# unibas-gravis/icp-proposal

Measured on AMD Instinct MI355X. Metric: ICP-proposal MH iterations/sec (femur GPMM r=50, ~50k-vtx target), higher is better.
Workload: dtype f64

## Files before the change

### icp-proposal_amd/csrc/icp_dense.hpp

```cpp
#pragma once
#include "icp_kernels.hpp"

namespace icp {

constexpr int kLdsDoubles = 18432;


__device__ __forceinline__ void write_corr(const CorrBuffers& cb, int k, int id, int aux, d3 pt, bool keep, d3 n,
                                           const Pose& pose, const double* __restrict__ ref, const double* __restrict__ mean) {
  double v0 = (pt.x - pose.t[0]) - pose.ctr[0], v1 = (pt.y - pose.t[1]) - pose.ctr[1], v2 = (pt.z - pose.t[2]) - pose.ctr[2];
  double b0 = ((pose.R[0] * v0 + pose.R[3] * v1) + pose.R[6] * v2) + pose.ctr[0];
  double b1 = ((pose.R[1] * v0 + pose.R[4] * v1) + pose.R[7] * v2) + pose.ctr[1];
  double b2 = ((pose.R[2] * v0 + pose.R[5] * v1) + pose.R[8] * v2) + pose.ctr[2];
  cb.id[k] = id;
  cb.aux[k] = aux;
  cb.pt[3 * k] = pt.x; cb.pt[3 * k + 1] = pt.y; cb.pt[3 * k + 2] = pt.z;
  cb.keep[k] = keep ? 1 : 0;
  cb.nhat[3 * k] = n.x; cb.nhat[3 * k + 1] = n.y; cb.nhat[3 * k + 2] = n.z;
  cb.e[3 * k] = (b0 - ref[3 * id]) - mean[3 * id];
  cb.e[3 * k + 1] = (b1 - ref[3 * id + 1]) - mean[3 * id + 1];
  cb.e[3 * k + 2] = (b2 - ref[3 * id + 2]) - mean[3 * id + 2];
}


__device__ __forceinline__ void correspond_model_one(const CorrTask& c, int k, d3 cp) {
  int aux = c.nnv ? c.nnv[k] : -1;
  bool on_boundary = (c.nnv && aux >= 0) ? c.boundary[aux] != 0 : false;
  d3 n = vertex_normal(c.x, c.tris, c.adj_off, c.adj, k);
  write_corr(c.cb, k, k, aux, cp, c.boundary_aware ? !on_boundary : true, n, c.pose, c.ref, c.mean);
}

__device__ __forceinline__ void correspond_target_one(const CorrTask& c, int k, int id) {
  bool on_boundary = c.boundary[id] != 0;
// ... 489 lines not shown
  const int tid = threadIdx.x, tw = 1 << tw_log2, ty = tid >> tw_log2, tx = tid & (tw - 1);
  const int rows = n + extra;
  for (int j = 0; j < n; ++j) {
    const double ajj = W[(size_t)j * ld + j];
    if (!(ajj > 0.0)) return false;
    const double inv = fast_rcp(ajj);
    for (int i = j + 1 + ty; i < rows; i += tw) {
      const double uij = W[(size_t)i * ld + j] * inv;
      const int kmax = i < n ? i : n - 1;
      for (int k = j + 1 + tx; k <= kmax; k += tw) W[(size_t)i * ld + k] = fma(-uij, W[(size_t)k * ld + j], W[(size_t)i * ld + k]);
    }
    __syncthreads();
  }
  return true;
}


#ifdef ICP_EIGEN_TIMING
extern __device__ long long g_eigen_stamps[64];
#define FAC_STAMP(i) do { if (threadIdx.x == 0 && blockIdx.x == 0) g_eigen_stamps[i] = __builtin_amdgcn_s_memrealtime(); } while (0)
#else
#define FAC_STAMP(i)
#endif

typedef double dense2 __attribute__((ext_vector_type(2)));

static __host__ __device__ inline int factor_tile_count(int r) {
  const int tr = (r + 2) >> 1;
  int c = 0;
  for (int t = 0; t < tr; ++t) c += (t >> 1) + 1;
  return c;
}

template <int TPT, int NT>
__device__ __forceinline__ bool factor_reg_body(int r, const double* __restrict__ Mpart, int S, double* __restrict__ M,
                                                double* __restrict__ alpha_out, int* __restrict__ status, int tail_base = -1,
                                                const double* __restrict__ tail_Ginv = nullptr, const double* __restrict__ Mplain = nullptr,
                                                bool solve = true) {
  __shared__ __attribute__((aligned(16))) double s_col[2][520];
  __shared__ double s_dinv[512], s_v[512];
  const int tid = threadIdx.x, n = r + 1;
  const int ld = r | 1;
  double* W = s_dyn;
  FAC_STAMP(16);
  constexpr int kGinvPer = 16;
  double ginv[kGinvPer];
  if (tail_base >= 0) {
#pragma unroll
    for (int u = 0; u < kGinvPer; ++u) {
      const int e = tid + u * NT;
      ginv[u] = e < r * r ? tail_Ginv[e] : 0.0;
    }
  }
  const int n_tiles = factor_tile_count(r);
  double v[TPT][2][4];
  int R0[TPT], C0[TPT];
#pragma unroll
  for (int t = 0; t < TPT; ++t) {
    const int e = tid + NT * t;
    int ti = 0, base = 0;
    if (e < n_tiles) {
      while (base + (ti >> 1) + 1 <= e) { base += (ti >> 1) + 1; ++ti; }
    }
    R0[t] = e < n_tiles ? 2 * ti : -2;
    C0[t] = e < n_tiles ? 4 * (e - base) : 0;
    bool live[2][4];
    size_t off[2][4];
// ... 23 lines not shown
#pragma unroll
      for (int u = 0; u < 4; ++u)
#pragma unroll
        for (int a = 0; a < 2; ++a)
#pragma unroll
          for (int c = 0; c < 4; ++c) p[u][a][c] = Mpart[(size_t)(sp + u) * nn + off[a][c]];
#pragma unroll
      for (int u = 0; u < 4; ++u)
#pragma unroll
        for (int a = 0; a < 2; ++a)
#pragma unroll
          for (int c = 0; c < 4; ++c) v[t][a][c] += p[u][a][c];
    }
    for (; sp < S; ++sp) {
      const double* P = Mpart + (size_t)sp * nn;
#pragma unroll
      for (int a = 0; a < 2; ++a)
#pragma unroll
        for (int c = 0; c < 4; ++c) v[t][a][c] += P[off[a][c]];
    }
#pragma unroll
    for (int a = 0; a < 2; ++a)
#pragma unroll
      for (int c = 0; c < 4; ++c) {
        const int i = R0[t] + a, k = C0[t] + c;
        double x = live[a][c] ? v[t][a][c] : 0.0;
        if (live[a][c]) {
          if (i < r && !Mplain) {
            if (i == k) x += 1.0;
            M[(size_t)i * r + k] = x;
            M[(size_t)k * r + i] = x;
            if (tail_base >= 0) { s_dyn[tail_base + i * ld + k] = x; s_dyn[tail_base + k * ld + i] = x; }
          }
          if (k == 0) { s_col[0][i] = x; W[(size_t)i * ld] = x; }
        }
        v[t][a][c] = x;
      }
  }
  if (tail_base >= 0) {
    const int offG = tail_base + r * ld;
#pragma unroll
    for (int u = 0; u < kGinvPer; ++u) {
      const int e = tid + u * NT;
      if (e < r * r) { const int i = e / r; s_dyn[offG + i * ld + (e - i * r)] = ginv[u]; }
    }
    for (int e = tid + kGinvPer * NT; e < r * r; e += NT) { const int i = e / r; s_dyn[offG + i * ld + (e - i * r)] = tail_Ginv[e]; }
  }
  __syncthreads();
  FAC_STAMP(17);
  bool ok = true;
  for (int j4 = 0; j4 < r && ok; j4 += 4) {
#pragma unroll
    for (int cc = 0; cc < 4; ++cc) {
      const int j = j4 + cc;
      if (j >= r) break;
      const double* cur = s_col[cc & 1];
      double* nxt = s_col[(cc + 1) & 1];
      const double ajj = cur[j];
      dense2 u[TPT], k01[TPT], k23[TPT];
#pragma unroll
      for (int t = 0; t < TPT; ++t) {
        const int rr = R0[t] < 0 ? 0 : R0[t];
        u[t] = *(const dense2*)&cur[rr];
        k01[t] = *(const dense2*)&cur[C0[t]];
        k23[t] = *(const dense2*)&cur[C0[t] + 2];
      }
      if (!(ajj > 0.0)) { ok = false; break; }
      const double inv = fast_rcp(ajj);
      const int kp = j + 1;
#pragma unroll
      for (int t = 0; t < TPT; ++t) {
        const double m0 = -(u[t].x * inv), m1 = -(u[t].y * inv);
        v[t][0][0] = fma(m0, k01[t].x, v[t][0][0]); v[t][0][1] = fma(m0, k01[t].y, v[t][0][1]);
        v[t][0][2] = fma(m0, k23[t].x, v[t][0][2]); v[t][0][3] = fma(m0, k23[t].y, v[t][0][3]);
        v[t][1][0] = fma(m1, k01[t].x, v[t][1][0]); v[t][1][1] = fma(m1, k01[t].y, v[t][1][1]);
        v[t][1][2] = fma(m1, k23[t].x, v[t][1][2]); v[t][1][3] = fma(m1, k23[t].y, v[t][1][3]);
        constexpr int cp = 0;
        (void)cp;
        if (kp < r && R0[t] >= 0 && C0[t] == (kp & ~3)) {
          const double p0 = v[t][0][(cc + 1) & 3], p1 = v[t][1][(cc + 1) & 3];
          *(dense2*)&nxt[R0[t]] = dense2{p0, p1};
          if (R0[t] >= kp && R0[t] < n) W[(size_t)R0[t] * ld + kp] = p0;
          if (R0[t] + 1 >= kp && R0[t] + 1 < n) W[(size_t)(R0[t] + 1) * ld + kp] = p1;
// ... 305 lines not shown
```

### icp-proposal_amd/csrc/icp_kernels.hpp

```cpp
#pragma once
#include <hip/hip_runtime.h>
#include <stdint.h>
#include "icp_device.hpp"

#include <cstdlib>
#include <vector>

namespace icp {

inline const char* dev_env(const char* name) {
#if defined(ICP_DEV_SWITCHES) || defined(ICP_TEST_HOOKS)
  return std::getenv(name);
#else
  (void)name;
  return nullptr;
#endif
}

constexpr int kBlock = 256;
__host__ __device__ static inline int cdiv(int a, int b) { return (a + b - 1) / b; }
static inline void set_dyn_lds(const void* fn, size_t bytes) {
  if (bytes > 48 * 1024) (void)hipFuncSetAttribute(fn, hipFuncAttributeMaxDynamicSharedMemorySize, (int)bytes);
}
static inline void set_dyn_lds_once(const void* fn, size_t max_bytes, bool* done) {
// ... 141 lines not shown
  const double* tpts;
  const unsigned char* boundary;
  const int* nnv;
  int boundary_aware;
  Pose pose;
  const double* ref;
  const double* mean;
  const int* tris;
  const int* adj_off;
  const int* adj;
  const double* cp = nullptr;
};

struct EntryInit { const double* coeffs_src = nullptr; double* coeffs_dst = nullptr; int r = 0; int* status = nullptr; };
void launch_correspond_model(hipStream_t st, int K, const double* x, const double* cp, const int* nnv,
                             const unsigned char* tgt_boundary, int boundary_aware, const Pose& pose,
                             const double* ref, const double* mean, const int* tris, const int* adj_off,
                             const int* adj, const CorrBuffers& cb, const EntryInit& init = EntryInit{});
void launch_correspond_target(hipStream_t st, int K, const double* x, const double* tpts, const int* nn_id,
                              const unsigned char* model_boundary, int boundary_aware, const Pose& pose,
                              const double* ref, const double* mean, const int* tris, const int* adj_off,
                              const int* adj, const CorrBuffers& cb, const EntryInit& init = EntryInit{});

int regression_splits(int K);
int regression_fold(int K, int r, int n_posteriors_in_launch);
int regression_macro(int r, int fold);
int regression_units(int r, int leaves, int fold, int macro);
void launch_regression(hipStream_t st, int K, int r, const double* Q, const CorrBuffers& cb, double w_tangent,
                       double kappa, double* Mpart, int* splits_out);

struct PosteriorFactorIO { const double* Mpart; int splits; double* M; double* alpha; int* status; double* scratch ;
                           double* Lout = nullptr; double* Sout = nullptr;  };
void launch_posterior_factor(hipStream_t st, int r, int n_post, const PosteriorFactorIO* io);
int posterior_factor_max();
void launch_sum_partials(hipStream_t st, int r, double* Mpart, int splits);
void launch_assemble_posterior_matrix(hipStream_t st, int r, const double* Mpart_summed, double* M);

struct TransitionTailIO {
  const double* alpha; const double* M; const double* c_from; const double* c_to; double step; double* out; int* status;
  const int* relay_in = nullptr; int* relay_out = nullptr;
};
void launch_transition_tails(hipStream_t st, int r, int n, const TransitionTailIO* io, const double* Ginv, double sigma2);
void launch_transition_tail_direct(hipStream_t st, int r, const TransitionTailIO& io, const double* G, double sigma2, double* work );

size_t eigen_work_doubles(int r);
constexpr int kEigenGaveUp = 3;
struct EigenSpec { int splits; const int* cancel; int seq; const int* ready; int ready_seq;
                   long long* wait_ticks = nullptr;  };
bool eigen_speculation_supported(int r);
struct EigenRequest { const double* M; const double* Vwarm; double* V; double* Vt; double* S; double* work; int* status;
                      const EigenSpec* spec; int* host_status; int* done_word; int done_value;
                      const double* sqrt_lambda = nullptr;
                      bool root = false;  };
constexpr int kEigenPairMax = 4;
bool launch_posterior_eigen_pair(hipStream_t st, int r, const double* sqrt_lambda, int n, const EigenRequest* rq);
struct EigenProblem {
  const double* M; const double* Vwarm ; double* Vout; double* Vtout; double* Sout; int* status;
  double* rotlog; int* meta; double* vpos; EigenSpec spec; int launch_id; int* host_status; int* done_word; int done_value;
  const double* sqrt_lambda;
};
EigenProblem eigen_problem_of(int r, const EigenRequest& rq);
void launch_posterior_eigen_resident(hipStream_t st, int r, int n, const EigenProblem* records, const int* skip, int root);
size_t eigen_many_record_bytes(int n);
int launch_posterior_eigen_many(hipStream_t st, int r, int n, const EigenRequest* rq, void* pinned_records, int* arrive);
void eigen_debug_dump(const double* work, int r);
void launch_posterior_eigen(hipStream_t st, int r, const double* M, const double* sqrt_lambda, const double* Vwarm, double* V,
// ... 724 lines not shown
```

### icp-proposal_amd/csrc/kernels_eigen.hip

```cpp
#include <algorithm>
#include <atomic>
#include <cstdio>
#include <cstdlib>

#include "icp_kernels.hpp"
#include "icp_dense.hpp"

namespace icp {

#ifdef ICP_EIGEN_TIMING
__device__ long long g_eigen_stamps[64];
#define EIG_STAMP(i) do { if (threadIdx.x == 0) g_eigen_stamps[i] = __builtin_amdgcn_s_memrealtime(); } while (0)
#else
#define EIG_STAMP(i)
#endif
}
#include "icp_tridiag.hpp"
namespace icp {

namespace {

constexpr int kEigenMaxSweeps = 40;
#ifndef ICP_LOOSE_TAU
#define ICP_LOOSE_TAU 5e-7
// ... 1372 lines not shown
  const EigenSpec spec = pb.spec;
  EIG_STAMP(0);
  if (tid == 0) s_cancel = 0;
  __syncthreads();
  if (tid == NT - 1) {
    if (spec.ready) {
      const long long t0 = __builtin_amdgcn_s_memrealtime();
      for (;;) {
        if (__hip_atomic_load(spec.ready, __ATOMIC_ACQUIRE, __HIP_MEMORY_SCOPE_AGENT) - spec.ready_seq >= 0) break;
        if (spec.cancel && __hip_atomic_load(spec.cancel, __ATOMIC_RELAXED, __HIP_MEMORY_SCOPE_SYSTEM) == spec.seq) { s_cancel = 1; break; }
        if (__builtin_amdgcn_s_memrealtime() - t0 > 500000) { s_cancel = 2; break; }
        __builtin_amdgcn_s_sleep(32);
      }
      if (spec.wait_ticks) atomicAdd((unsigned long long*)spec.wait_ticks, (unsigned long long)(__builtin_amdgcn_s_memrealtime() - t0));
    } else if (spec.cancel) {
      if (__hip_atomic_load(spec.cancel, __ATOMIC_RELAXED, __HIP_MEMORY_SCOPE_SYSTEM) == spec.seq) s_cancel = 1;
    }
  }
  __syncthreads();
  __builtin_amdgcn_fence(__ATOMIC_ACQUIRE, "agent");
  if (s_cancel) {
    if (tid == 0) {
      if (s_cancel == 2) {
        if (pb.host_status) __hip_atomic_store(pb.host_status, kEigenGaveUp, __ATOMIC_RELAXED, __HIP_MEMORY_SCOPE_SYSTEM);
        pb.Vout[0] = __builtin_nan("");
      }
      __threadfence();
      if (pb.done_word) __hip_atomic_store(pb.done_word, pb.done_value, __ATOMIC_RELEASE, __HIP_MEMORY_SCOPE_AGENT);
    }
    return;
  }
  EIG_STAMP(1);
  double* scratch = pb.rotlog;
  const bool ok = factor_reg_body<1, NT>(r, pb.M, spec.splits, scratch, scratch + (size_t)r * r, (int*)(scratch + (size_t)r * r + r),
                                         -1, nullptr, spec.splits > 0 ? nullptr : pb.M, false);
  EIG_STAMP(3);
  const int ld = r | 1;
  const double* W = s_dyn;
  if (ok) {
    for (int e = tid; e < r * r; e += NT) {
      const int i = e / r, k = e - i * r;
      const double v = k <= i ? W[(size_t)i * ld + k] * fast_rsqrt(W[(size_t)k * ld + k]) : 0.0;
      pb.Vout[(size_t)i * r + k] = v;
      pb.Vtout[(size_t)k * r + i] = v;
    }
    if (tid < r) pb.Sout[tid] = fast_rsqrt(W[(size_t)tid * ld + tid]);
  }
  EIG_STAMP(4);
  if (tid == 0) {
    pb.status[0] = ok ? 0 : 2; pb.status[-1] = 0;
    if (pb.host_status) __hip_atomic_store(pb.host_status, ok ? 0 : 2, __ATOMIC_RELAXED, __HIP_MEMORY_SCOPE_SYSTEM);
  }
  __threadfence();
  __syncthreads();
  if (tid == 0 && pb.done_word) __hip_atomic_store(pb.done_word, pb.done_value, __ATOMIC_RELEASE, __HIP_MEMORY_SCOPE_AGENT);
  EIG_STAMP(5);
}

namespace {
template <class Batch>
void launch_root_batch(hipStream_t st, int r, int n, const Batch& batch) {
  ProfScope _ps(st, KID_EIGEN);
  const size_t shmem = sizeof(double) * (size_t)(r + 1) * (r | 1);
  if (factor_tile_count(r) <= 256) {
    set_dyn_lds((const void*)k_posterior_root<Batch, 256>, shmem);
    hipLaunchKernelGGL((k_posterior_root<Batch, 256>), dim3(n), dim3(256), shmem, st, r, batch);
  } else {
// ... 94 lines not shown
```

### icp-proposal_amd/csrc/kernels_factor.hip

```cpp
#include <algorithm>

#include "icp_kernels.hpp"
#include "icp_dense.hpp"

namespace icp {

namespace {

struct FactorArgs {
  const double* Mpart[kFactorMax];
  int splits[kFactorMax];
  double* M[kFactorMax];
  double* alpha[kFactorMax];
  int* status[kFactorMax];
  double* scratch[kFactorMax];
  double* Lout[kFactorMax];
  double* Sout[kFactorMax];
};

__device__ __forceinline__ void emit_factor_rootfree(int r, const double* W, int ld, double* __restrict__ Lout, double* __restrict__ Sout) {
  for (int e = threadIdx.x; e < r * r; e += blockDim.x) {
    const int i = e / r, j = e - i * r;
    double v = 0.0;
    if (j <= i) {
// ... 35 lines not shown
  for (int j = tid; j < r; j += nt) {
    const double d = fast_rsqrt(W[(size_t)j * ld + j]);
    s_dinv[j] = d;
    s_v[j] = W[(size_t)r * ld + j] * d;
  }
  __syncthreads();
  if (r <= 64) {
    if (tid < 64) {
      const int i = tid;
      double v = i < r ? s_v[i] : 0.0;
      const double di = i < r ? s_dinv[i] : 0.0;
      for (int j = r - 1; j >= 0; --j) {
        const double xj = __shfl(v, j, 64) * s_dinv[j];
        if (i == j) v = xj;
        else if (i < j) v = fma(-(W[(size_t)j * ld + i] * di), xj, v);
      }
      if (i < r) fa.alpha[p][i] = v;
    }
  } else {
    for (int j = r - 1; j >= 0; --j) {
      if (tid == 0) s_v[j] = s_v[j] * s_dinv[j];
      __syncthreads();
      const double xj = s_v[j];
      for (int i = tid; i < j; i += nt) s_v[i] = fma(-(W[(size_t)j * ld + i] * s_dinv[i]), xj, s_v[i]);
      __syncthreads();
    }
    for (int i = tid; i < r; i += nt) fa.alpha[p][i] = s_v[i];
  }
}

template <int TPT, int NT>
__global__ void __launch_bounds__(NT) k_posterior_factor_reg(int r, FactorArgs fa) {
  const int p = blockIdx.x;
  const bool ok = factor_reg_body<TPT, NT>(r, fa.Mpart[p], fa.splits[p], fa.M[p], fa.alpha[p], fa.status[p]);
  if (ok && fa.Lout[p]) emit_factor_rootfree(r, s_dyn, r | 1, fa.Lout[p], fa.Sout[p]);
}

constexpr int kCholNB = 64;
constexpr int kCholMaxRank = 256;

__device__ __forceinline__ void factor_backsolve_emit(int r, const double* __restrict__ W, double* D, double* s_y, double* s_part,
                                                      const FactorArgs& fa, int p) {
  const int tid = threadIdx.x, nt = blockDim.x;
  constexpr int ldd = kCholNB + 1;
  for (int j = tid; j < r; j += nt) s_y[j] = W[(size_t)r * r + j];
  const int last_kb = ((r - 1) / kCholNB) * kCholNB;
  for (int kb = last_kb; kb >= 0; kb -= kCholNB) {
    const int nbk = min(kCholNB, r - kb);
    for (int e = tid; e < kCholNB * kCholNB; e += nt) {
      const int i = e >> 6, j = e & 63;
      if (j <= i && i < nbk) D[i * ldd + j] = W[(size_t)(kb + i) * r + kb + j];
    }
    __syncthreads();
    if (tid < 64) {
      const int i = tid, ic = i < nbk ? i : nbk - 1;
      double x = s_y[kb + ic];
      const double di = fast_rcp(D[ic * ldd + ic]);
      constexpr int kA = 4;
      double lq[kA];
#pragma unroll
      for (int a = 0; a < kA; ++a) lq[a] = D[max(nbk - 1 - a, ic) * ldd + ic];
      for (int j0 = nbk - 1; j0 >= 0; j0 -= kA) {
#pragma unroll
        for (int a = 0; a < kA; ++a) {
          const int j = j0 - a;
          const double lij = lq[a];
          lq[a] = D[max(j - kA, ic) * ldd + ic];
// ... 195 lines not shown
```

### icp-proposal_amd/csrc/kernels_step.hip

```cpp
#include <algorithm>
#include <cstddef>
#include <cstdlib>
#include <cstring>

#include "icp_kernels.hpp"
#include "icp_search.hpp"
#include "icp_dense.hpp"
#include "../../include/icp_sincos.h"

namespace icp {

namespace {

constexpr int kStepBlock = 256;

__device__ __forceinline__ void step_begin_body(const StepBeginArgs& a, const int bx) {
  __shared__ double s_c[512];
  const int tid = threadIdx.x, r = a.r;
  const double* zsrc = r <= kStepInlineZ ? a.zin : a.z_ptr;
  if (a.wait_flag || a.wait2_flag) {
    if (tid == 0) {
      const long long t0 = __builtin_amdgcn_s_memrealtime();
      for (;;) {
        const bool ok1 = !a.wait_flag || __hip_atomic_load(a.wait_flag, __ATOMIC_ACQUIRE, __HIP_MEMORY_SCOPE_AGENT) - a.wait_seq >= 0;
// ... 458 lines not shown
  } else {
    if (a.reduce_kind == 1) {
      if (a.Kred > 0) sum_gauss_logpdf_body(a.Kred, a.d2, a.mean, a.sigma, a.red_out);
      if (a.Kred2 > 0) { __syncthreads(); sum_gauss_logpdf_body(a.Kred2, a.d2b, a.mean, a.sigma, a.red_out + 4); }
    } else if (a.reduce_kind == 2) {
      if (a.Kred > 0) dist_stats_body(a.Kred, a.d2, a.red_out);
      if (a.Kred2 > 0) { __syncthreads(); dist_stats_body(a.Kred2, a.d2b, a.red_out + 4); }
    }
  }
}
__device__ __forceinline__ int step_regression_grid(const StepRegressionArgs& a) {
  return step_regression_blocks(a.ustart[a.n]) + (a.reduce_kind ? 1 : 0);
}

__global__ void __launch_bounds__(kStepBlock) k_step_regression(StepRegressionArgs a) { step_regression_body(a, blockIdx.x); }

__global__ void __launch_bounds__(256) k_step_reduce(StepReduceArgs a) {
  const int which = blockIdx.y, e = blockIdx.x * 256 + threadIdx.x;
  if (which >= a.n || e >= a.nn) return;
  double* P = a.Mpart[which];
  const int S = a.splits[which];
  double acc = 0.0;
  for (int s0 = 0; s0 < S; s0 += 8) {
    double q[8];
#pragma unroll
    for (int u = 0; u < 8; ++u) q[u] = P[(size_t)min(s0 + u, S - 1) * a.nn + e];
#pragma unroll
    for (int u = 0; u < 8; ++u) if (s0 + u < S) acc += q[u];
  }
  P[e] = acc;
}


template <int E, int NT>
__device__ __forceinline__ void step_finish_body(const StepFinishArgs& a, const int b) {
  if (b == 0 && threadIdx.x == 0 && a.ready_flag) __hip_atomic_store(a.ready_flag, a.seq, __ATOMIC_RELEASE, __HIP_MEMORY_SCOPE_AGENT);
  if (b < a.n) {
    const bool ok = factor_reg_body<E, NT>(a.r, a.Mpart[b], a.splits[b], a.M[b], a.alpha[b], a.status[b], a.tail_base, a.Ginv);
    if (threadIdx.x == 0) a.host_status[b][0] = ok ? 0 : 1;
    if (ok) {
      __syncthreads();
      const TransitionTailIO& t = a.bwd[b];
      tail_body(a.r, t.alpha, t.M, t.c_from, t.c_to, t.step, t.out, t.status, a.Ginv, a.sigma2, a.n_lds, a.tpr_log2,
                a.tail_base >= 0 ? a.tail_base : 0, a.tail_base >= 0);
    } else if (threadIdx.x == 0) {
      a.bwd[b].out[0] = __builtin_nan("");
      a.bwd[b].status[0] = 0;
    }
  } else {
    const TransitionTailIO& t = a.fwd[b - a.n];
    tail_body(a.r, t.alpha, t.M, t.c_from, t.c_to, t.step, t.out, t.status, a.Ginv, a.sigma2, a.n_lds, a.tpr_log2);
  }
  __syncthreads();
  if (threadIdx.x == 0) {
    __threadfence_system();
    if (atomicAdd(a.done_counter, 1) == 2 * a.n - 1) {
      *a.done_counter = 0;
      __hip_atomic_store(a.host_flag, a.seq, __ATOMIC_RELAXED, __HIP_MEMORY_SCOPE_SYSTEM);
    }
  }
}

template <int E, int NT>
__global__ void __launch_bounds__(NT) k_step_finish(StepFinishArgs a) { step_finish_body<E, NT>(a, blockIdx.x); }


__global__ void __launch_bounds__(256) k_step_batch_args(const uint4* __restrict__ src, uint4* __restrict__ dst, int n16, StepBatchGate gate) {
  const int i = blockIdx.x * 256 + threadIdx.x;
  if (i < n16) dst[i] = src[i];
  if (gate.counter && blockIdx.x == 0 && threadIdx.x == 0) {
    const long long t0 = __builtin_amdgcn_s_memrealtime();
    while (__hip_atomic_load(gate.counter, __ATOMIC_RELAXED, __HIP_MEMORY_SCOPE_AGENT) - gate.expected < 0) {
      if (__builtin_amdgcn_s_memrealtime() - t0 > 200000000ll) {
        __hip_atomic_store(gate.error, 1, __ATOMIC_RELAXED, __HIP_MEMORY_SCOPE_SYSTEM);
        break;
      }
      __builtin_amdgcn_s_sleep(4);
    }
  }
}

__global__ void __launch_bounds__(kStepBlock) k_step_begin_batch(const StepBeginArgs* __restrict__ batch) {
  const StepBeginArgs& a = batch[blockIdx.y];
  if ((int)blockIdx.x >= step_begin_grid(a)) return;
  step_begin_body(a, blockIdx.x);
}
template <int RMAX>
__global__ void __launch_bounds__(kStepBlock) k_step_begin_batch_reg(const StepBeginArgs* __restrict__ batch) {
  const StepBeginArgs& a = batch[blockIdx.y];
  if ((int)blockIdx.x >= step_begin_grid(a)) return;
  step_begin_body_reg<RMAX>(a, blockIdx.x);
}
template <bool kPrepared>
__global__ void __launch_bounds__(kSearchBlock, kPrepared ? 8 : 1) k_step_filter_batch(const StepSearchArgs* __restrict__ batch) {
  const StepSearchArgs& a = batch[blockIdx.y];
  if ((int)blockIdx.x >= a.fstart[a.n_surf + a.n_vert]) return;
  step_filter_body<kPrepared>(a, blockIdx.x);
}
__global__ void __launch_bounds__(64) k_step_resolve_batch(const StepSearchArgs* __restrict__ batch) {
  const StepSearchArgs& a = batch[blockIdx.y];
  if ((int)blockIdx.x >= a.rstart[a.n_surf + a.n_vert]) return;
  step_resolve_body(a, blockIdx.x);
}
__global__ void __launch_bounds__(kStepBlock) k_step_regression_batch(const StepRegressionArgs* __restrict__ batch) {
  const StepRegressionArgs& a = batch[blockIdx.y];
  if ((int)blockIdx.x >= step_regression_grid(a)) return;
  step_regression_body(a, blockIdx.x);
}
__global__ void __launch_bounds__(kStepBlock) k_step_regression_batch_fold(const StepRegressionArgs* __restrict__ batch) {
  const StepRegressionArgs& a = batch[blockIdx.y];
  if ((int)blockIdx.x >= step_regression_grid(a)) return;
  step_regression_body<true>(a, blockIdx.x);
}
template <int E, int NT>
__global__ void __launch_bounds__(NT) k_step_finish_batch(const StepFinishArgs* __restrict__ batch) {
  const StepFinishArgs& a = batch[blockIdx.y];
  if ((int)blockIdx.x >= 2 * a.n) return;
  step_finish_body<E, NT>(a, blockIdx.x);
}


__global__ void __launch_bounds__(kStepBlock) k_step_begin_twin(StepTwin<StepBeginArgs> t) {
  const StepBeginArgs& a = t.a[blockIdx.y];
  if ((int)blockIdx.x >= step_begin_grid(a)) return;
  step_begin_body(a, blockIdx.x);
}
template <int RMAX>
__global__ void __launch_bounds__(kStepBlock) k_step_begin_twin_reg(StepTwin<StepBeginArgs> t) {
  const StepBeginArgs& a = t.a[blockIdx.y];
  if ((int)blockIdx.x >= step_begin_grid(a)) return;
  step_begin_body_reg<RMAX>(a, blockIdx.x);
}
__global__ void __launch_bounds__(kSearchBlock) k_step_filter_twin(StepTwin<StepSearchArgs> t) {
  const StepSearchArgs& a = t.a[blockIdx.y];
  if ((int)blockIdx.x >= a.fstart[a.n_surf + a.n_vert]) return;
  step_filter_body(a, blockIdx.x);
}
__global__ void __launch_bounds__(64) k_step_resolve_twin(StepTwin<StepSearchArgs> t) {
  const StepSearchArgs& a = t.a[blockIdx.y];
  if ((int)blockIdx.x >= a.rstart[a.n_surf + a.n_vert]) return;
  step_resolve_body(a, blockIdx.x);
}
__global__ void __launch_bounds__(64) k_step_search_twin(StepTwin<StepOneSearchArgs> t) {
  const StepOneSearchArgs& o = t.a[blockIdx.y];
  if ((int)blockIdx.x >= o.a.rstart[o.a.n_surf + o.a.n_vert]) return;
  step_search_body(o, blockIdx.x);
}
__global__ void __launch_bounds__(kStepBlock) k_step_regression_twin(StepTwin<StepRegressionArgs> t) {
  const StepRegressionArgs& a = t.a[blockIdx.y];
  if ((int)blockIdx.x >= step_regression_grid(a)) return;
  step_regression_body(a, blockIdx.x);
}
template <int E, int NT>
__global__ void __launch_bounds__(NT) k_step_finish_twin(StepTwin<StepFinishArgs> t) {
  const StepFinishArgs& a = t.a[blockIdx.y];
  if ((int)blockIdx.x >= 2 * a.n) return;
  step_finish_body<E, NT>(a, blockIdx.x);
}

thread_local StepCapture* t_capture = nullptr;

struct FinishPlan { int E , NT, n_lds, tail_base; size_t shmem; bool ok; };

FinishPlan finish_plan(int r) {
  FinishPlan p{0, 0, 0, -1, 0, false};
  const int ld = r | 1;
  const size_t tiles = (size_t)factor_tile_count(r);
  const size_t w = (size_t)(r + 1) * ld, one = (size_t)r * ld;
  const size_t budget = (size_t)kLdsDoubles - 4700;
  if (w > budget) return p;
  if (tiles <= 256) { p.E = 1; p.NT = 256; }
  else if (tiles <= 1024) { p.E = 2; p.NT = 512; }
  else if (tiles <= 2048) { p.E = 2; p.NT = 1024; }
  else return p;
  p.n_lds = 2 * one <= budget ? 2 : (one <= budget ? 1 : 0);
  const size_t tails = one * p.n_lds;
  if (p.n_lds == 2 && w + tails <= budget) { p.tail_base = (int)w; p.shmem = sizeof(double) * (w + tails); }
  else p.shmem = sizeof(double) * (w > tails ? w : tails);
  p.ok = true;
  return p;
}

template <int E, int NT>
void launch_finish(hipStream_t st, const StepFinishArgs& a, size_t shmem) {
  static size_t lds_granted = 0;
  if (shmem > lds_granted) { set_dyn_lds((const void*)k_step_finish<E, NT>, shmem); lds_granted = shmem; }
  hipLaunchKernelGGL((k_step_finish<E, NT>), dim3(2 * a.n), dim3(NT), shmem, st, a);
}

}

bool step_finish_supported(int r) { return finish_plan(r).ok; }

void launch_step_begin(hipStream_t st, const StepBeginArgs& a_in) {
  StepBeginArgs a = a_in;
  a.inst_blocks = cdiv(a.N, kStepBeginPoints);
  const int vblocks = cdiv(std::max(a.has_vert ? a.vert.Kpad : 0, a.n_zero2), kStepBlock);
  if (t_capture) { t_capture->begin = a; t_capture->grid[0] = a.inst_blocks + vblocks; return; }
  ProfScope _ps(st, KID_STEP_BEGIN);
  static const bool no_reg = dev_env("ICP_BEGIN_STREAMED") != nullptr;
  if (a.hold_regs && a.r >= 32 && a.r <= 52 && !no_reg) hipLaunchKernelGGL(k_step_begin_reg<52>, dim3(a.inst_blocks + vblocks), dim3(kStepBlock), 0, st, a);
  else if (a.hold_regs && a.r >= 32 && a.r <= 64 && !no_reg) hipLaunchKernelGGL(k_step_begin_reg<64>, dim3(a.inst_blocks + vblocks), dim3(kStepBlock), 0, st, a);
  else hipLaunchKernelGGL(k_step_begin, dim3(a.inst_blocks + vblocks), dim3(kStepBlock), 0, st, a);
}

void launch_step_filter(hipStream_t st, const StepSearchArgs& a) {
  const int grid = a.fstart[a.n_surf + a.n_vert];
  if (t_capture) { t_capture->search = a; t_capture->grid[1] = grid; t_capture->tables = TargetTables{}; return; }
  if (grid <= 0) return;
  ProfScope _ps(st, KID_STEP_FILTER);
  hipLaunchKernelGGL(k_step_filter, dim3(grid), dim3(kSearchBlock), 0, st, a);
}

void launch_step_resolve(hipStream_t st, const StepSearchArgs& a) {
  const int grid = a.rstart[a.n_surf + a.n_vert];
  if (t_capture) { t_capture->grid[2] = grid; return; }
  if (grid <= 0) return;
  ProfScope _ps(st, KID_STEP_RESOLVE);
  hipLaunchKernelGGL(k_step_resolve, dim3(grid), dim3(64), 0, st, a);
}

void launch_step_search(hipStream_t st, const StepSearchArgs& a, const TargetTables& t) {
  const int grid = a.rstart[a.n_surf + a.n_vert];
  if (t_capture) { t_capture->search = a; t_capture->tables = t; t_capture->grid[1] = 0; t_capture->grid[2] = grid; return; }
  if (grid <= 0) return;
  ProfScope _ps(st, KID_STEP_SEARCH);
  hipLaunchKernelGGL(k_step_search, dim3(grid), dim3(64), 0, st, StepOneSearchArgs{a, t});
}

void launch_step_regression(hipStream_t st, const StepRegressionArgs& a) {
  const int blocks = step_regression_blocks(a.ustart[a.n]) + (a.reduce_kind ? 1 : 0);
  if (t_capture) { t_capture->regression = a; t_capture->grid[3] = blocks; return; }
  if (blocks <= 0) return;
  ProfScope _ps(st, KID_STEP_REGRESSION);
  hipLaunchKernelGGL(k_step_regression, dim3(blocks), dim3(kStepBlock), 0, st, a);
}

void launch_step_reduce(hipStream_t st, const StepReduceArgs& a) {
  if (t_capture) return;
  ProfScope _ps(st, KID_STEP_REGRESSION);
  hipLaunchKernelGGL(k_step_reduce, dim3(cdiv(a.nn, 256), a.n), dim3(256), 0, st, a);
}

namespace {
StepFinishArgs finish_args_final(const StepFinishArgs& a_in, const FinishPlan& p) {
  StepFinishArgs a = a_in;
  a.n_lds = p.n_lds;
  a.tail_base = p.tail_base;
  a.tpr_log2 = matvec_tpr_log2(a.r, a.r <= 64 ? 256 : p.NT);
  return a;
}
template <int E, int NT>
void launch_finish_twin(hipStream_t st, const StepTwin<StepFinishArgs>& t, int gx, size_t shmem) {
  static size_t lds_granted = 0;
  if (shmem > lds_granted) { set_dyn_lds((const void*)k_step_finish_twin<E, NT>, shmem); lds_granted = shmem; }
  hipLaunchKernelGGL((k_step_finish_twin<E, NT>), dim3(gx, 2), dim3(NT), shmem, st, t);
}
}

void launch_step_twin_front(hipStream_t st, const StepCapture& l0, const StepCapture& l1) {
  {
    StepTwin<StepBeginArgs> t;
    t.a[0] = l0.begin; t.a[1] = l1.begin;
    const dim3 grid(std::max(l0.grid[0], l1.grid[0]), 2);
    ProfScope _ps(st, KID_STEP_BEGIN);
    static const bool no_reg = dev_env("ICP_BEGIN_STREAMED") != nullptr;
    const int r = l0.begin.r;
    const bool hold = l0.begin.hold_regs && l1.begin.hold_regs && !no_reg;
    if (hold && r >= 32 && r <= 52) hipLaunchKernelGGL(k_step_begin_twin_reg<52>, grid, dim3(kStepBlock), 0, st, t);
    else if (hold && r >= 32 && r <= 64) hipLaunchKernelGGL(k_step_begin_twin_reg<64>, grid, dim3(kStepBlock), 0, st, t);
    else hipLaunchKernelGGL(k_step_begin_twin, grid, dim3(kStepBlock), 0, st, t);
  }
  const bool one_search = l0.tables.balls != nullptr && l1.tables.balls != nullptr;
  StepTwin<StepSearchArgs> q;
  q.a[0] = l0.search; q.a[1] = l1.search;
  if (const int gx = std::max(l0.grid[2], l1.grid[2]); one_search && gx > 0) {
    StepTwin<StepOneSearchArgs> o;
    o.a[0] = StepOneSearchArgs{l0.search, l0.tables}; o.a[1] = StepOneSearchArgs{l1.search, l1.tables};
    ProfScope _ps(st, KID_STEP_SEARCH);
    hipLaunchKernelGGL(k_step_search_twin, dim3(gx, 2), dim3(64), 0, st, o);
  }
  if (const int gx = std::max(l0.grid[1], l1.grid[1]); !one_search && gx > 0) {
    ProfScope _ps(st, KID_STEP_FILTER);
    hipLaunchKernelGGL(k_step_filter_twin, dim3(gx, 2), dim3(kSearchBlock), 0, st, q);
  }
  if (const int gx = std::max(l0.grid[2], l1.grid[2]); !one_search && gx > 0) {
    ProfScope _ps(st, KID_STEP_RESOLVE);
    hipLaunchKernelGGL(k_step_resolve_twin, dim3(gx, 2), dim3(64), 0, st, q);
  }
  if (const int gx = std::max(l0.grid[3], l1.grid[3]); gx > 0) {
    StepTwin<StepRegressionArgs> g;
    g.a[0] = l0.regression; g.a[1] = l1.regression;
    ProfScope _ps(st, KID_STEP_REGRESSION);
    hipLaunchKernelGGL(k_step_regression_twin, dim3(gx, 2), dim3(kStepBlock), 0, st, g);
  }
}

void launch_step_twin_finish(hipStream_t st, const StepFinishArgs& l0, const StepFinishArgs& l1) {
  const FinishPlan p = finish_plan(l0.r);
  StepTwin<StepFinishArgs> t;
  t.a[0] = finish_args_final(l0, p);
  t.a[1] = finish_args_final(l1, p);
  t.a[1].ready_flag = nullptr;
  const int gx = 2 * std::max(l0.n, l1.n);
  ProfScope _ps(st, KID_STEP_FINISH);
  if (p.E == 1 && p.NT == 256) launch_finish_twin<1, 256>(st, t, gx, p.shmem);
  else if (p.E == 2 && p.NT == 512) launch_finish_twin<2, 512>(st, t, gx, p.shmem);
  else launch_finish_twin<2, 1024>(st, t, gx, p.shmem);
}

void launch_step_finish(hipStream_t st, const StepFinishArgs& a_in) {
  const FinishPlan p = finish_plan(a_in.r);
  const StepFinishArgs a = finish_args_final(a_in, p);
  if (t_capture) { t_capture->finish = a; t_capture->grid[4] = 2 * a.n; return; }
  ProfScope _ps(st, KID_STEP_FINISH);
  if (p.E == 1 && p.NT == 256) launch_finish<1, 256>(st, a, p.shmem);
  else if (p.E == 2 && p.NT == 512) launch_finish<2, 512>(st, a, p.shmem);
  else launch_finish<2, 1024>(st, a, p.shmem);
}


void step_capture(StepCapture* c) { t_capture = c; }

namespace {
template <int E, int NT>
void launch_finish_batch(hipStream_t st, const StepFinishArgs* batch, int gx, int B, size_t shmem) {
  static size_t lds_granted = 0;
  if (shmem > lds_granted) { set_dyn_lds((const void*)k_step_finish_batch<E, NT>, shmem); lds_granted = shmem; }
  hipLaunchKernelGGL((k_step_finish_batch<E, NT>), dim3(gx, B), dim3(NT), shmem, st, batch);
}
inline size_t up16(size_t x) { return (x + 15) & ~(size_t)15; }
}

void launch_step_batch_resident(hipStream_t st, int B, const int gx[5], int r, const StepBeginArgs* begin, const StepSearchArgs* search,
                                const StepRegressionArgs* regression, const StepFinishArgs* finish, bool filter_prepared, bool reg_folded) {
  if (B <= 0) return;
  if (gx[0] > 0) { ProfScope _ps(st, KID_STEP_BEGIN); hipLaunchKernelGGL(k_step_begin_batch, dim3(gx[0], B), dim3(kStepBlock), 0, st, begin); }
  if (gx[1] > 0) {
    ProfScope _ps(st, KID_STEP_FILTER);
    if (filter_prepared) hipLaunchKernelGGL(k_step_filter_batch<true>, dim3(gx[1], B), dim3(kSearchBlock), 0, st, search);
    else hipLaunchKernelGGL(k_step_filter_batch<false>, dim3(gx[1], B), dim3(kSearchBlock), 0, st, search);
  }
  if (gx[2] > 0) { ProfScope _ps(st, KID_STEP_RESOLVE); hipLaunchKernelGGL(k_step_resolve_batch, dim3(gx[2], B), dim3(64), 0, st, search); }
  if (gx[3] > 0) {
    ProfScope _ps(st, KID_STEP_REGRESSION);
    if (reg_folded) hipLaunchKernelGGL(k_step_regression_batch_fold, dim3(gx[3], B), dim3(kStepBlock), 0, st, regression);
    else hipLaunchKernelGGL(k_step_regression_batch, dim3(gx[3], B), dim3(kStepBlock), 0, st, regression);
  }
  if (gx[4] > 0) {
    ProfScope _ps(st, KID_STEP_FINISH);
    const FinishPlan p = finish_plan(r);
    if (p.E == 1 && p.NT == 256) launch_finish_batch<1, 256>(st, finish, gx[4], B, p.shmem);
    else if (p.E == 2 && p.NT == 512) launch_finish_batch<2, 512>(st, finish, gx[4], B, p.shmem);
    else launch_finish_batch<2, 1024>(st, finish, gx[4], B, p.shmem);
  }
}


namespace {
__device__ __forceinline__ unsigned long long mh_splitmix64(unsigned long long x) {
  x += 0x9E3779B97F4A7C15ull;
  x = (x ^ (x >> 30)) * 0xBF58476D1CE4E5B9ull;
  x = (x ^ (x >> 27)) * 0x94D049BB133111EBull;
  return x ^ (x >> 31);
}
__device__ __forceinline__ double mh_uniform(unsigned long long seed, unsigned long long step, unsigned long long lane) {
  const unsigned long long h = mh_splitmix64(mh_splitmix64(mh_splitmix64(seed) ^ (step * 0xD1342543DE82EF95ull)) ^ (lane * 0x2545F4914F6CDD1Dull));
  return ((double)(h >> 11) + 0.5) * (1.0 / 9007199254740992.0);
}
__device__ __forceinline__ int mh_pick(int n, const double* w, double u) {
  double acc = 0.0;
  for (int i = 0; i < n; ++i) {
    acc += w[i];
    if (acc >= u) return i;
  }
  return n - 1;
}
__device__ __forceinline__ double mh_lse(int n, const double* w, const double* t) {
  double mx = -__builtin_inf();
  for (int i = 0; i < n; ++i)
    if (t[i] > mx) mx = t[i];
  if (mx == -__builtin_inf()) return mx;
  double s = 0.0;
  for (int i = 0; i < n; ++i) s += w[i] * exp(t[i] - mx);
  return log(s) + mx;
}
template <class T>
// ... 403 lines not shown
    static const bool no_reg = dev_env("ICP_BEGIN_STREAMED") != nullptr;
    const int r = caps[0].begin.r;
    bool hold = false;
    for (int b = 0; b < B; ++b) hold = hold || caps[b].begin.hold_regs != 0;
    if (hold && r >= 32 && r <= 52 && !no_reg) hipLaunchKernelGGL(k_step_begin_batch_reg<52>, dim3(gx[0], B), dim3(kStepBlock), 0, st, (const StepBeginArgs*)d);
    else if (hold && r >= 32 && r <= 64 && !no_reg) hipLaunchKernelGGL(k_step_begin_batch_reg<64>, dim3(gx[0], B), dim3(kStepBlock), 0, st, (const StepBeginArgs*)d);
    else hipLaunchKernelGGL(k_step_begin_batch, dim3(gx[0], B), dim3(kStepBlock), 0, st, (const StepBeginArgs*)d);
  }
  if (gx[1] > 0) {
    ProfScope _ps(st, KID_STEP_FILTER);
    bool prepared = true;
    for (int b = 0; b < B; ++b) prepared = prepared && step_filter_prepared(caps[b].search);
    if (prepared) hipLaunchKernelGGL(k_step_filter_batch<true>, dim3(gx[1], B), dim3(kSearchBlock), 0, st, (const StepSearchArgs*)(d + o1));
    else hipLaunchKernelGGL(k_step_filter_batch<false>, dim3(gx[1], B), dim3(kSearchBlock), 0, st, (const StepSearchArgs*)(d + o1));
  }
  if (gx[2] > 0) { ProfScope _ps(st, KID_STEP_RESOLVE); hipLaunchKernelGGL(k_step_resolve_batch, dim3(gx[2], B), dim3(64), 0, st, (const StepSearchArgs*)(d + o1)); }
  if (gx[3] > 0) {
    ProfScope _ps(st, KID_STEP_REGRESSION);
    bool reg_folded = false;
    for (int b = 0; b < B; ++b)
      for (int i = 0; i < caps[b].regression.n && i < 2; ++i) reg_folded = reg_folded || caps[b].regression.fold[i] > 1;
    if (reg_folded) hipLaunchKernelGGL(k_step_regression_batch_fold, dim3(gx[3], B), dim3(kStepBlock), 0, st, (const StepRegressionArgs*)(d + o2));
    else hipLaunchKernelGGL(k_step_regression_batch, dim3(gx[3], B), dim3(kStepBlock), 0, st, (const StepRegressionArgs*)(d + o2));
  }
  if (gx[4] > 0) {
    const FinishPlan p = finish_plan(caps[0].finish.r);
    if (st_finish && st_finish != st && ev) {
      (void)hipEventRecord(ev, st);
      (void)hipStreamWaitEvent(st_finish, ev, 0);
      st = st_finish;
    }
    ProfScope _ps(st, KID_STEP_FINISH);
    const StepFinishArgs* fb = (const StepFinishArgs*)(d + o3);
    if (p.E == 1 && p.NT == 256) launch_finish_batch<1, 256>(st, fb, gx[4], B, p.shmem);
    else if (p.E == 2 && p.NT == 512) launch_finish_batch<2, 512>(st, fb, gx[4], B, p.shmem);
    else launch_finish_batch<2, 1024>(st, fb, gx[4], B, p.shmem);
  }
}

}
```

Baseline: 13410.

## Use 4-column panel Cholesky updates in step-finish factorization

Adds a panel-width-4 path to the register-tiled Cholesky in the finish kernel. Each thread derives the 4x4 pivot block itself and applies all four column eliminations in registers, so there is one __syncthreads per four columns instead of per-column exchanges through shared memory. The next panel's four columns are published into a strided LDS buffer. It becomes the default for the E=1/256 and E=2/512 plans (a thread-local flag keeps the old column path), at the cost of redundant pivot math in every thread and higher register use.

```diff
diff --git a/icp-proposal_amd/csrc/icp_dense.hpp b/icp-proposal_amd/csrc/icp_dense.hpp
--- a/icp-proposal_amd/csrc/icp_dense.hpp
+++ b/icp-proposal_amd/csrc/icp_dense.hpp
@@ -1,4 +1,6 @@
 #pragma once
+#include <type_traits>
+
 #include "icp_kernels.hpp"
 
 namespace icp {
@@ -554,7 +556,38 @@
   return c;
 }
 
-template <int TPT, int NT>
+struct PanelPivots { double e10, e20, e30, e21, e31, e32, d[4], inv[4]; };
+
+__device__ __forceinline__ void panel_row(const PanelPivots& p, double (&x)[4], double (&m)[4]) {
+  m[0] = -(x[0] * p.inv[0]);
+  x[1] = fma(m[0], p.e10, x[1]); x[2] = fma(m[0], p.e20, x[2]); x[3] = fma(m[0], p.e30, x[3]);
+  m[1] = -(x[1] * p.inv[1]);
+  x[2] = fma(m[1], p.e21, x[2]); x[3] = fma(m[1], p.e31, x[3]);
+  m[2] = -(x[2] * p.inv[2]);
+  x[3] = fma(m[2], p.e32, x[3]);
+  m[3] = -(x[3] * p.inv[3]);
+}
+constexpr int kPanelStride = 130;
+__device__ __forceinline__ void panel_load2(const double* pan, int row, double (&x)[2][4]) {
+#pragma unroll
+  for (int s = 0; s < 4; ++s) {
+    const dense2 q = *(const dense2*)&pan[s * kPanelStride + row];
+    x[0][s] = q.x; x[1][s] = q.y;
+  }
+}
+__device__ __forceinline__ void panel_load4(const double* pan, int row, double (&x)[4][4]) {
+#pragma unroll
+  for (int s = 0; s < 4; ++s) {
+    const dense2 lo = *(const dense2*)&pan[s * kPanelStride + row], hi = *(const dense2*)&pan[s * kPanelStride + row + 2];
+    x[0][s] = lo.x; x[1][s] = lo.y; x[2][s] = hi.x; x[3][s] = hi.y;
+  }
+}
+__device__ __forceinline__ void panel_publish(double* pan, int row, const double (&v)[2][4]) {
+#pragma unroll
+  for (int s = 0; s < 4; ++s) *(dense2*)&pan[s * kPanelStride + row] = dense2{v[0][s], v[1][s]};
+}
+
+template <int TPT, int NT, int PW>
 __device__ __forceinline__ bool factor_reg_body(int r, const double* __restrict__ Mpart, int S, double* __restrict__ M,
                                                 double* __restrict__ alpha_out, int* __restrict__ status, int tail_base = -1,
                                                 const double* __restrict__ tail_Ginv = nullptr, const double* __restrict__ Mplain = nullptr,
@@ -644,10 +677,11 @@
             M[(size_t)k * r + i] = x;
             if (tail_base >= 0) { s_dyn[tail_base + i * ld + k] = x; s_dyn[tail_base + k * ld + i] = x; }
           }
-          if (k == 0) { s_col[0][i] = x; W[(size_t)i * ld] = x; }
+          if (k == 0) { if (PW == 1) s_col[0][i] = x; W[(size_t)i * ld] = x; }
         }
         v[t][a][c] = x;
       }
+    if (PW == 4 && R0[t] >= 0 && C0[t] == 0) panel_publish(s_col[0], R0[t], v[t]);
   }
   if (tail_base >= 0) {
     const int offG = tail_base + r * ld;
@@ -661,6 +695,79 @@
   __syncthreads();
   FAC_STAMP(17);
   bool ok = true;
+  if constexpr (PW == 4) {
+    auto panel = [&](auto kFull, const int J, const int nc) {
+      const double* cur = s_col[(J >> 2) & 1];
+      double* nxt = s_col[((J >> 2) + 1) & 1];
+      double pr[4][4], xr[TPT][2][4], k[TPT][4][4];
+      bool live[TPT];
+      panel_load4(cur, J, pr);
+#pragma unroll
+      for (int t = 0; t < TPT; ++t) {
+        live[t] = R0[t] >= 0 && C0[t] >= J;
+        if (live[t]) {
+          panel_load2(cur, R0[t], xr[t]);
+          panel_load4(cur, C0[t], k[t]);
+        }
+      }
+      PanelPivots pv;
+      pv.d[0] = pr[0][0];
+      pv.inv[0] = fast_rcp(pv.d[0]);
+      pv.e10 = pr[1][0]; pv.e20 = pr[2][0]; pv.e30 = pr[3][0];
+      const double m10 = -(pv.e10 * pv.inv[0]), m20 = -(pv.e20 * pv.inv[0]), m30 = -(pv.e30 * pv.inv[0]);
+      pv.d[1] = fma(m10, pv.e10, pr[1][1]);
+      pv.e21 = fma(m20, pv.e10, pr[2][1]); pv.e31 = fma(m30, pv.e10, pr[3][1]);
+      const double x22 = fma(m20, pv.e20, pr[2][2]), x32 = fma(m30, pv.e20, pr[3][2]), x33 = fma(m30, pv.e30, pr[3][3]);
+      pv.inv[1] = fast_rcp(pv.d[1]);
+      const double m21 = -(pv.e21 * pv.inv[1]), m31 = -(pv.e31 * pv.inv[1]);
+      pv.d[2] = fma(m21, pv.e21, x22);
+      pv.e32 = fma(m31, pv.e21, x32);
+      const double x33b = fma(m31, pv.e31, x33);
+      pv.inv[2] = fast_rcp(pv.d[2]);
+      const double m32 = -(pv.e32 * pv.inv[2]);
+      pv.d[3] = fma(m32, pv.e32, x33b);
+      pv.inv[3] = fast_rcp(pv.d[3]);
+#pragma unroll
+      for (int t = 0; t < TPT; ++t) {
+        if (!live[t]) continue;
+        double m[2][4], mm[4];
+#pragma unroll
+        for (int a = 0; a < 2; ++a) panel_row(pv, xr[t][a], m[a]);
+#pragma unroll
+        for (int c = 0; c < 4; ++c) panel_row(pv, k[t][c], mm);
+        const bool owner = C0[t] == J;
+#pragma unroll
+        for (int s = 0; s < 4; ++s) {
+          if (!decltype(kFull)::value && s >= nc) break;
+          if (s > 0 && owner) {
+#pragma unroll
+            for (int a = 0; a < 2; ++a)
+              if (R0[t] + a >= J + s && R0[t] + a < n) W[(size_t)(R0[t] + a) * ld + J + s] = v[t][a][s];
+          }
+#pragma unroll
+          for (int a = 0; a < 2; ++a)
+#pragma unroll
+            for (int c = 0; c < 4; ++c) v[t][a][c] = fma(m[a][s], k[t][c][s], v[t][a][c]);
+        }
+        if (decltype(kFull)::value && C0[t] == J + 4 && J + 4 < r) {
+          panel_publish(nxt, R0[t], v[t]);
+#pragma unroll
+          for (int a = 0; a < 2; ++a)
+            if (R0[t] + a >= J + 4 && R0[t] + a < n) W[(size_t)(R0[t] + a) * ld + J + 4] = v[t][a][0];
+        }
+      }
+      bool good = true;
+#pragma unroll
+      for (int s = 0; s < 4; ++s)
+        if ((decltype(kFull)::value || s < nc) && !(pv.d[s] > 0.0)) good = false;
+      return good;
+    };
+    for (int J = 0; J < r && ok; J += 4) {
+      ok = r - J >= 4 ? panel(std::true_type{}, J, 4) : panel(std::false_type{}, J, r - J);
+      if (!ok) break;
+      __syncthreads();
+    }
+  } else
   for (int j4 = 0; j4 < r && ok; j4 += 4) {
 #pragma unroll
     for (int cc = 0; cc < 4; ++cc) {
diff --git a/icp-proposal_amd/csrc/icp_kernels.hpp b/icp-proposal_amd/csrc/icp_kernels.hpp
--- a/icp-proposal_amd/csrc/icp_kernels.hpp
+++ b/icp-proposal_amd/csrc/icp_kernels.hpp
@@ -197,6 +197,8 @@
 struct PosteriorFactorIO { const double* Mpart; int splits; double* M; double* alpha; int* status; double* scratch ;
                            double* Lout = nullptr; double* Sout = nullptr;  };
 void launch_posterior_factor(hipStream_t st, int r, int n_post, const PosteriorFactorIO* io);
+extern thread_local bool g_factor_columns;
+inline bool factor_columns() { return g_factor_columns; }
 int posterior_factor_max();
 void launch_sum_partials(hipStream_t st, int r, double* Mpart, int splits);
 void launch_assemble_posterior_matrix(hipStream_t st, int r, const double* Mpart_summed, double* M);
diff --git a/icp-proposal_amd/csrc/kernels_eigen.hip b/icp-proposal_amd/csrc/kernels_eigen.hip
--- a/icp-proposal_amd/csrc/kernels_eigen.hip
+++ b/icp-proposal_amd/csrc/kernels_eigen.hip
@@ -1428,7 +1428,7 @@
   }
   EIG_STAMP(1);
   double* scratch = pb.rotlog;
-  const bool ok = factor_reg_body<1, NT>(r, pb.M, spec.splits, scratch, scratch + (size_t)r * r, (int*)(scratch + (size_t)r * r + r),
+  const bool ok = factor_reg_body<1, NT, 1>(r, pb.M, spec.splits, scratch, scratch + (size_t)r * r, (int*)(scratch + (size_t)r * r + r),
                                          -1, nullptr, spec.splits > 0 ? nullptr : pb.M, false);
   EIG_STAMP(3);
   const int ld = r | 1;
diff --git a/icp-proposal_amd/csrc/kernels_factor.hip b/icp-proposal_amd/csrc/kernels_factor.hip
--- a/icp-proposal_amd/csrc/kernels_factor.hip
+++ b/icp-proposal_amd/csrc/kernels_factor.hip
@@ -91,7 +91,7 @@
 template <int TPT, int NT>
 __global__ void __launch_bounds__(NT) k_posterior_factor_reg(int r, FactorArgs fa) {
   const int p = blockIdx.x;
-  const bool ok = factor_reg_body<TPT, NT>(r, fa.Mpart[p], fa.splits[p], fa.M[p], fa.alpha[p], fa.status[p]);
+  const bool ok = factor_reg_body<TPT, NT, 1>(r, fa.Mpart[p], fa.splits[p], fa.M[p], fa.alpha[p], fa.status[p]);
   if (ok && fa.Lout[p]) emit_factor_rootfree(r, s_dyn, r | 1, fa.Lout[p], fa.Sout[p]);
 }
 
diff --git a/icp-proposal_amd/csrc/kernels_step.hip b/icp-proposal_amd/csrc/kernels_step.hip
--- a/icp-proposal_amd/csrc/kernels_step.hip
+++ b/icp-proposal_amd/csrc/kernels_step.hip
@@ -514,11 +514,11 @@
 }
 
 
-template <int E, int NT>
+template <int E, int NT, int PW>
 __device__ __forceinline__ void step_finish_body(const StepFinishArgs& a, const int b) {
   if (b == 0 && threadIdx.x == 0 && a.ready_flag) __hip_atomic_store(a.ready_flag, a.seq, __ATOMIC_RELEASE, __HIP_MEMORY_SCOPE_AGENT);
   if (b < a.n) {
-    const bool ok = factor_reg_body<E, NT>(a.r, a.Mpart[b], a.splits[b], a.M[b], a.alpha[b], a.status[b], a.tail_base, a.Ginv);
+    const bool ok = factor_reg_body<E, NT, PW>(a.r, a.Mpart[b], a.splits[b], a.M[b], a.alpha[b], a.status[b], a.tail_base, a.Ginv);
     if (threadIdx.x == 0) a.host_status[b][0] = ok ? 0 : 1;
     if (ok) {
       __syncthreads();
@@ -543,8 +543,8 @@
   }
 }
 
-template <int E, int NT>
-__global__ void __launch_bounds__(NT) k_step_finish(StepFinishArgs a) { step_finish_body<E, NT>(a, blockIdx.x); }
+template <int E, int NT, int PW>
+__global__ void __launch_bounds__(NT) k_step_finish(StepFinishArgs a) { step_finish_body<E, NT, PW>(a, blockIdx.x); }
 
 
 __global__ void __launch_bounds__(256) k_step_batch_args(const uint4* __restrict__ src, uint4* __restrict__ dst, int n16, StepBatchGate gate) {
@@ -594,11 +594,11 @@
   if ((int)blockIdx.x >= step_regression_grid(a)) return;
   step_regression_body<true>(a, blockIdx.x);
 }
-template <int E, int NT>
+template <int E, int NT, int PW>
 __global__ void __launch_bounds__(NT) k_step_finish_batch(const StepFinishArgs* __restrict__ batch) {
   const StepFinishArgs& a = batch[blockIdx.y];
   if ((int)blockIdx.x >= 2 * a.n) return;
-  step_finish_body<E, NT>(a, blockIdx.x);
+  step_finish_body<E, NT, PW>(a, blockIdx.x);
 }
 
 
@@ -633,11 +633,11 @@
   if ((int)blockIdx.x >= step_regression_grid(a)) return;
   step_regression_body(a, blockIdx.x);
 }
-template <int E, int NT>
+template <int E, int NT, int PW>
 __global__ void __launch_bounds__(NT) k_step_finish_twin(StepTwin<StepFinishArgs> t) {
   const StepFinishArgs& a = t.a[blockIdx.y];
   if ((int)blockIdx.x >= 2 * a.n) return;
-  step_finish_body<E, NT>(a, blockIdx.x);
+  step_finish_body<E, NT, PW>(a, blockIdx.x);
 }
 
 thread_local StepCapture* t_capture = nullptr;
@@ -663,14 +663,25 @@
   return p;
 }
 
-template <int E, int NT>
+template <int E_, int NT_, int PW_> struct FinishKind { static constexpr int E = E_, NT = NT_, PW = PW_; };
+template <class F>
+void finish_dispatch(const FinishPlan& p, F&& f) {
+  const bool cols = factor_columns();
+  if (p.E == 1 && p.NT == 256) { if (cols) f(FinishKind<1, 256, 1>{}); else f(FinishKind<1, 256, 4>{}); }
+  else if (p.E == 2 && p.NT == 512) { if (cols) f(FinishKind<2, 512, 1>{}); else f(FinishKind<2, 512, 4>{}); }
+  else f(FinishKind<2, 1024, 1>{});
+}
+
+template <int E, int NT, int PW>
 void launch_finish(hipStream_t st, const StepFinishArgs& a, size_t shmem) {
   static size_t lds_granted = 0;
-  if (shmem > lds_granted) { set_dyn_lds((const void*)k_step_finish<E, NT>, shmem); lds_granted = shmem; }
-  hipLaunchKernelGGL((k_step_finish<E, NT>), dim3(2 * a.n), dim3(NT), shmem, st, a);
-}
-
-}
+  if (shmem > lds_granted) { set_dyn_lds((const void*)k_step_finish<E, NT, PW>, shmem); lds_granted = shmem; }
+  hipLaunchKernelGGL((k_step_finish<E, NT, PW>), dim3(2 * a.n), dim3(NT), shmem, st, a);
+}
+
+}
+
+thread_local bool g_factor_columns = false;
 
 bool step_finish_supported(int r) { return finish_plan(r).ok; }
 
@@ -732,11 +743,11 @@
   a.tpr_log2 = matvec_tpr_log2(a.r, a.r <= 64 ? 256 : p.NT);
   return a;
 }
-template <int E, int NT>
+template <int E, int NT, int PW>
 void launch_finish_twin(hipStream_t st, const StepTwin<StepFinishArgs>& t, int gx, size_t shmem) {
   static size_t lds_granted = 0;
-  if (shmem > lds_granted) { set_dyn_lds((const void*)k_step_finish_twin<E, NT>, shmem); lds_granted = shmem; }
-  hipLaunchKernelGGL((k_step_finish_twin<E, NT>), dim3(gx, 2), dim3(NT), shmem, st, t);
+  if (shmem > lds_granted) { set_dyn_lds((const void*)k_step_finish_twin<E, NT, PW>, shmem); lds_granted = shmem; }
+  hipLaunchKernelGGL((k_step_finish_twin<E, NT, PW>), dim3(gx, 2), dim3(NT), shmem, st, t);
 }
 }
 
@@ -786,9 +797,7 @@
   t.a[1].ready_flag = nullptr;
   const int gx = 2 * std::max(l0.n, l1.n);
   ProfScope _ps(st, KID_STEP_FINISH);
-  if (p.E == 1 && p.NT == 256) launch_finish_twin<1, 256>(st, t, gx, p.shmem);
-  else if (p.E == 2 && p.NT == 512) launch_finish_twin<2, 512>(st, t, gx, p.shmem);
-  else launch_finish_twin<2, 1024>(st, t, gx, p.shmem);
+  finish_dispatch(p, [&](auto k) { launch_finish_twin<decltype(k)::E, decltype(k)::NT, decltype(k)::PW>(st, t, gx, p.shmem); });
 }
 
 void launch_step_finish(hipStream_t st, const StepFinishArgs& a_in) {
@@ -796,20 +805,18 @@
   const StepFinishArgs a = finish_args_final(a_in, p);
   if (t_capture) { t_capture->finish = a; t_capture->grid[4] = 2 * a.n; return; }
   ProfScope _ps(st, KID_STEP_FINISH);
-  if (p.E == 1 && p.NT == 256) launch_finish<1, 256>(st, a, p.shmem);
-  else if (p.E == 2 && p.NT == 512) launch_finish<2, 512>(st, a, p.shmem);
-  else launch_finish<2, 1024>(st, a, p.shmem);
+  finish_dispatch(p, [&](auto k) { launch_finish<decltype(k)::E, decltype(k)::NT, decltype(k)::PW>(st, a, p.shmem); });
 }
 
 
 void step_capture(StepCapture* c) { t_capture = c; }
 
 namespace {
-template <int E, int NT>
+template <int E, int NT, int PW>
 void launch_finish_batch(hipStream_t st, const StepFinishArgs* batch, int gx, int B, size_t shmem) {
   static size_t lds_granted = 0;
-  if (shmem > lds_granted) { set_dyn_lds((const void*)k_step_finish_batch<E, NT>, shmem); lds_granted = shmem; }
-  hipLaunchKernelGGL((k_step_finish_batch<E, NT>), dim3(gx, B), dim3(NT), shmem, st, batch);
+  if (shmem > lds_granted) { set_dyn_lds((const void*)k_step_finish_batch<E, NT, PW>, shmem); lds_granted = shmem; }
+  hipLaunchKernelGGL((k_step_finish_batch<E, NT, PW>), dim3(gx, B), dim3(NT), shmem, st, batch);
 }
 inline size_t up16(size_t x) { return (x + 15) & ~(size_t)15; }
 }
@@ -832,9 +839,7 @@
   if (gx[4] > 0) {
     ProfScope _ps(st, KID_STEP_FINISH);
     const FinishPlan p = finish_plan(r);
-    if (p.E == 1 && p.NT == 256) launch_finish_batch<1, 256>(st, finish, gx[4], B, p.shmem);
-    else if (p.E == 2 && p.NT == 512) launch_finish_batch<2, 512>(st, finish, gx[4], B, p.shmem);
-    else launch_finish_batch<2, 1024>(st, finish, gx[4], B, p.shmem);
+    finish_dispatch(p, [&](auto k) { launch_finish_batch<decltype(k)::E, decltype(k)::NT, decltype(k)::PW>(st, finish, gx[4], B, p.shmem); });
   }
 }
 
@@ -1304,10 +1309,8 @@
     }
     ProfScope _ps(st, KID_STEP_FINISH);
     const StepFinishArgs* fb = (const StepFinishArgs*)(d + o3);
-    if (p.E == 1 && p.NT == 256) launch_finish_batch<1, 256>(st, fb, gx[4], B, p.shmem);
-    else if (p.E == 2 && p.NT == 512) launch_finish_batch<2, 512>(st, fb, gx[4], B, p.shmem);
-    else launch_finish_batch<2, 1024>(st, fb, gx[4], B, p.shmem);
-  }
-}
-
-}
+    finish_dispatch(p, [&](auto k) { launch_finish_batch<decltype(k)::E, decltype(k)::NT, decltype(k)::PW>(st, fb, gx[4], B, p.shmem); });
+  }
+}
+
+}
```

Result: no change. 13470 (median of 2 runs) (+0.4%).
